# MartijnAB/guacamole

Measured on AMD Instinct MI355X. Metric: pileup loci/sec at 30x WGS; achieved HBM GB/s vs roofline, higher is better.
Workload: dtype u8; 1 GPU; germline-threshold, synthetic 30x chr20-length shard per GPU (configs[1]); genome_loci=63025519, visited_loci_per_gpu=63025483, reads_per_gpu=12612887, contigs_per_gpu=1, read_len=150, threshold=8, parallelism=loci-sharded x1

## Files before the change

guacamole_amd/csrc/gq_germline_direct.h:

```cpp
#pragma once

#include "gq_kernels.h"


#ifndef GQ_DIR_WPE
#define GQ_DIR_WPE 4
#endif
#ifndef GQ_DIR_MASKED
#define GQ_DIR_MASKED 0
#endif
#ifndef GQ_DIR_EVPF
#define GQ_DIR_EVPF 0
#endif
#ifndef GQ_DIR_U
#define GQ_DIR_U 4
#endif
struct DirCfg {
  static constexpr int kT = 512;
  static constexpr int kWaves = 4;
  static constexpr int kThreads = 64 * kWaves;
  static constexpr int kU = GQ_DIR_U;
  static constexpr int kRound = 64;
  static constexpr int kSlots = 256;
  static constexpr int64_t kMaxWin = 65535;
  static constexpr int64_t kShallow = 255;
};


template <bool DEEP>
__global__ __launch_bounds__(DirCfg::kThreads) __attribute__((amdgpu_waves_per_eu(GQ_DIR_WPE))) void germline_direct(
    const Tile *__restrict__ tiles, int64_t n_tiles, DevReads R, int threshold, int emit_ref, int emit_no_call,
    CallRec *__restrict__ recs, ComplexItem *__restrict__ cplx, OutGeom og, Counters *ctr, int32_t *__restrict__ slow,
    int32_t *__restrict__ deep, int dbg) {
  using C = DirCfg;
  constexpr int T = C::kT, U = C::kU;
  constexpr int EW = DEEP ? 2 * T : T;
  __shared__ __attribute__((aligned(16))) uint32_t evw[C::kWaves][EW];
  __shared__ __attribute__((aligned(16))) uint32_t mkw[C::kWaves][T];
  __shared__ __attribute__((aligned(16))) uint32_t dlw[C::kWaves][T];
  __shared__ __attribute__((aligned(16))) uint2 rcw[C::kWaves][C::kSlots];
  __shared__ int32_t hxw[C::kWaves][64], hnw[C::kWaves][64];
  __shared__ unsigned outn[2];
  const int lane = threadIdx.x & 63;
  const int wave = __builtin_amdgcn_readfirstlane((int)(threadIdx.x >> 6));
  uint32_t *ev = evw[wave], *mk = mkw[wave], *dl = dlw[wave];
  uint2 *rc = rcw[wave];
  int32_t *hx = hxw[wave], *hn = hnw[wave];
  auto ix = [](int32_t x) { return ((x & 7) << 6) | (x >> 3); };
  auto zero_words = [&]() {
    const uint4 z4 = make_uint4(0u, 0u, 0u, 0u);
    uint4 *e4 = reinterpret_cast<uint4 *>(ev), *m4 = reinterpret_cast<uint4 *>(mk), *d4 = reinterpret_cast<uint4 *>(dl);
#pragma unroll
    for (int q = 0; q < EW / 256; ++q) e4[64 * q + lane] = z4;
    m4[lane] = z4; m4[64 + lane] = z4; d4[lane] = z4; d4[64 + lane] = z4;
  };
  zero_words();
  if (threadIdx.x < 2) outn[threadIdx.x] = 0;
  __syncthreads();
  const int64_t per = n_tiles / gridDim.x, extra = n_tiles % gridDim.x;
  const int64_t i0 = blockIdx.x * per + min((int64_t)blockIdx.x, extra);
  const int64_t i1 = i0 + per + ((int64_t)blockIdx.x < extra ? 1 : 0);
  const int part = DEEP ? kPartsCols + (int)((blockIdx.x * C::kWaves + wave) & (kPartsWalk - 1)) : (int)blockIdx.x;
  const unsigned long long obase[2] = {og.slot(0, part, 0), og.slot(1, part, 0)};
  const unsigned long long ocap[2] = {og.cap(0, part), og.cap(1, part)};
  auto reserve = [&](int which, unsigned n) -> unsigned long long {
    return DEEP ? wave_reserve(&ctr->part[which][part], n) : (unsigned long long)wave_reserve_lds_n(outn + which, n);
  };
  unsigned visited = 0, amb = 0, ties = 0;
  uint64_t clk[8] = {0, 0, 0, 0, 0, 0, 0, 0};
  const bool multi_sample = R.n_samples > 1;
  const int64_t thr1 = (int64_t)threshold + 1;
  const uint32_t thr1u = (uint32_t)(thr1 < 0 ? 0 : thr1 > 101 ? 101 : thr1);
  const uint32_t thr1b = thr1u & 0xFFu;
  auto passes = [=](uint32_t count, uint32_t depth) { return (count & 0xFFFFu) * 100u >= thr1b * (depth & 0xFFFFu); };
  const __amdgpu_buffer_rsrc_t trs =
      __builtin_amdgcn_make_buffer_rsrc((void *)tiles, (short)0, (int)(64 * n_tiles), 0x00020000);
  const uint32_t tvo = lane < 16 ? 4u * (uint32_t)lane : 0x80000000u;
  auto fetch = [&](int64_t t) -> uint32_t { return __builtin_amdgcn_raw_buffer_load_b32(trs, (int)tvo, (int)(64 * t), 0); };
  auto f32 = [](uint32_t rec, int d) { return (uint32_t)__builtin_amdgcn_readlane((int)rec, d); };
  auto f64 = [&](uint32_t rec, int d) { return (int64_t)((uint64_t)f32(rec, d) | ((uint64_t)f32(rec, d + 1) << 32)); };
  const int32_t colr = 8 * lane;
  const int64_t n_deep = DEEP ? (int64_t)min(ctr->n_deep, (unsigned long long)n_tiles) : 0;
  const int64_t iend = DEEP ? n_deep : i1, istep = DEEP ? (int64_t)gridDim.x * C::kWaves : C::kWaves;
  int64_t i = DEEP ? (int64_t)blockIdx.x * C::kWaves + wave : i0 + wave;
  for (; i < iend; i += istep) {
    const uint64_t t_a = (dbg & 16) ? __builtin_readcyclecounter() : 0;
    const int64_t tid = DEEP ? (int64_t)__builtin_amdgcn_readfirstlane(deep[i]) : i;
    const uint32_t rec = fetch(tid);
    const int64_t ord0 = f64(rec, 0);
    const int32_t tcontig = (int32_t)f32(rec, 6);
    const int32_t L0 = (int32_t)f32(rec, 7), L1 = (int32_t)f32(rec, 8);
    const int64_t rb = f64(rec, 2), re = f64(rec, 4);
    const int32_t B0 = L0 & ~(T - 1);
    const int32_t col = B0 + colr;
    if (re <= rb) continue;
    if (re - rb > C::kMaxWin) {
      if (lane == 0) slow[atomicAdd(&ctr->n_slow, 1ull)] = (int32_t)tid;
      continue;
    }
    if (!DEEP && re - rb > C::kShallow) {
      if (lane == 0) deep[atomicAdd(&ctr->n_deep, 1ull)] = (int32_t)tid;
      continue;
    }
    uint32_t ca[2] = {0, 0}, cc[2] = {0, 0}, ct[2] = {0, 0}, cg[2] = {0, 0}, cn[2] = {0, 0};
    uint32_t wA[4] = {0, 0, 0, 0}, wC[4] = {0, 0, 0, 0}, wT[4] = {0, 0, 0, 0}, wG[4] = {0, 0, 0, 0},
             wN[4] = {0, 0, 0, 0};
    uint32_t nac[2] = {0, 0}, ntg[2] = {0, 0};
    int nn = 0, since = 0;
    auto fold = [&]() {
#pragma unroll
      for (int h = 0; h < 2; ++h) {
        ca[h] += nac[h] & 0x0F0F0F0Fu;
        cc[h] += (nac[h] >> 4) & 0x0F0F0F0Fu;
        ct[h] += ntg[h] & 0x0F0F0F0Fu;
        cg[h] += (ntg[h] >> 4) & 0x0F0F0F0Fu;
        nac[h] = ntg[h] = 0;
      }
      nn = 0;
    };
    auto widen = [&]() {
      if (!DEEP) return;
      auto w2 = [](uint32_t (&w)[4], uint32_t (&c)[2]) {
#pragma unroll
        for (int h = 0; h < 2; ++h) {
          w[2 * h] += __builtin_amdgcn_perm(0u, c[h], 0x0c010c00u);
          w[2 * h + 1] += __builtin_amdgcn_perm(0u, c[h], 0x0c030c02u);
          c[h] = 0;
        }
      };
      w2(wA, ca);
      w2(wC, cc);
      w2(wT, ct);
      w2(wG, cg);
      w2(wN, cn);
    };
    bool bad = false;
    uint32_t badb = 0;
    const uint64_t t_b = (dbg & 16) ? __builtin_readcyclecounter() : 0;
    struct Fields {
      int32_t s, e, nmd, ld;
      int64_t so, mo;
    };
    auto load_fields = [&](int64_t c0) {
      Fields f{0, 0, 0, 0, 0, 0};
      const int64_t r = c0 + lane;
      if (r < re) {
        f.s = R.start[r];
        f.e = R.end[r];
        f.so = R.seq_off[r];
        f.ld = R.lead[r];
        f.nmd = R.n_md[r];
        f.mo = R.md_off[r];
      }
      return f;
    };
    int64_t tbase = 0;
    bool defer = false;
    __amdgpu_buffer_rsrc_t srs;
    Fields nf = load_fields(rb);
    int64_t c0 = rb;
    bool first_round = true;
    uint32_t pv4[4] = {0u, 0u, 0u, 0u};
    int64_t pv_c0 = -1;
    while (c0 < re) {
      const uint64_t t_round = (dbg & 16) ? __builtin_readcyclecounter() : 0;
      hx[lane] = -1;
      hn[lane] = 0x7FFFFFFF;
      int32_t nslot = 0;
      while (c0 < re) {
        const uint64_t t_rd = (dbg & 16) ? __builtin_readcyclecounter() : 0;
        const int64_t r = c0 + lane;
        const bool valid = r < re;
        const Fields f = nf;
        const int32_t s = f.s, e = f.e, nmd = f.nmd, ld = f.ld;
        const int64_t so = f.so, mo = f.mo;
        const bool nomd = valid && nmd < 0;
        const bool gen = valid && !nomd && ld < 0;
        uint32_t nrun = valid && !nomd && !gen && e > B0 && s < B0 + T ? 1u : 0u;
        const bool evr = valid && !nomd && nmd > 0 && s < B0 + T && !(dbg & 64);
        uint32_t v4[4] = {0u, 0u, 0u, 0u};
        auto load_ev = [&](int32_t k0) {
#pragma unroll
          for (int j = 0; j < 4; ++j) v4[j] = R.md_ev[mo + (k0 + j < nmd ? k0 + j : nmd - 1)];
        };
        auto ev_add = [&](int32_t l, uint8_t base) {
          const int cat = base_cat(base);
          if (cat < 4) {
            const int32_t x = ix(l - B0);
            if (DEEP) atomicAdd(&ev[(cat >> 1) * T + x], 1u << (16 * (cat & 1)));
            else atomicAdd(&ev[x], 1u << (8 * cat));
          }
        };
        if (evr) {
          if (GQ_DIR_EVPF && pv_c0 == c0) {
#pragma unroll
            for (int j = 0; j < 4; ++j) v4[j] = pv4[j];
          } else {
            load_ev(0);
          }
        }
        if (gen && e > B0 && s < B0 + T) nrun = (uint32_t)min(-1 - ld, C::kSlots);
        const uint32_t incl = wave_incl_scan(nrun);
        const int32_t total = (int32_t)__builtin_amdgcn_readlane((int)incl, 63);
        const uint64_t t_f = (dbg & 16) ? __builtin_readcyclecounter() : 0;
        if (nslot > 0 && nslot + total > C::kSlots) break;
        if (total > C::kSlots) {
          bad = true;
          c0 = re;
          break;
        }
        if (c0 + C::kRound < re) nf = load_fields(c0 + C::kRound);
        if (first_round) {
          int64_t so_min = valid ? so : INT64_MAX;
#pragma unroll
          for (int d = 1; d < 64; d <<= 1) {
            const int64_t o = __shfl_xor(so_min, d, 64);
            so_min = o < so_min ? o : so_min;
          }
          const bool headed = R.seq_head >= 8 && so_min >= 0;
          defer = !DEEP && so_min < 8 && !headed;
          tbase = so_min >= 8 || headed ? so_min - 8 : 0;
          tbase = (int64_t)(((uint64_t)(uint32_t)__builtin_amdgcn_readfirstlane((int)(uint32_t)((uint64_t)tbase >> 32)) << 32) |
                            (uint32_t)__builtin_amdgcn_readfirstlane((int)(uint32_t)(uint64_t)tbase));
          const int64_t span = R.seq_cap - tbase;
          srs = __builtin_amdgcn_make_buffer_rsrc((void *)(R.seq + tbase), (short)0,
                                                  (int)(span < 0x7FFFFFFF ? span : 0x7FFFFFFF), 0x00020000);
          first_round = false;
        }
        bad = bad || nomd ||
              (valid && (so < tbase || so + (ld > 0 ? ld : 0) + (e > s ? e - s : 0) + 16384 + 1024 - tbase >= 0x7FFFFFF0ll));
        int32_t slot = nslot + (int32_t)(incl - nrun);
        auto put = [&](int32_t a, int32_t b, int64_t p) {
          const int32_t s16 = min(max(a - B0, -32768), 32767), e16 = min(max(b - B0, -32768), 32767);
          const int32_t K = (int32_t)(p - tbase - (int64_t)(a - B0));
          rc[slot] = make_uint2((uint32_t)(uint16_t)s16 | ((uint32_t)(uint16_t)e16 << 16), (uint32_t)K);
          atomicMax(&hx[min(max(s16, 0), T - 1) >> 3], slot);
          atomicMin(&hn[min(max(e16 - 1, 0), T - 1) >> 3], slot);
          ++slot;
// ... 323 lines not shown
```

guacamole_amd/csrc/gq_host.h:

```cpp
#pragma once
#include <hip/hip_runtime.h>

#include <algorithm>
#include <cstddef>
#include <cstring>
#include <condition_variable>
#include <mutex>
#include <thread>
#include <cstdarg>
#include <cstdio>
#include <string>
#include <utility>
#include <vector>

#include "../../include/gqpileup.h"
#include "gq_kernels.h"

namespace gq {

gq_status set_err(gq_status s, const char *fmt, ...);

#define HIP_TRY(expr)                                                                         \
  do {                                                                                        \
    hipError_t _e = (expr);                                                                   \
    if (_e != hipSuccess)                                                                     \
      return set_err(GQ_E_HIP, "%s failed: %s (%s:%d)", #expr, hipGetErrorString(_e), __FILE__, __LINE__); \
  } while (0)

constexpr int kBlock = 256;
constexpr int kGermT = 512;
constexpr int kCountT = 512;
constexpr size_t kSeqPad = 2048;

constexpr size_t kSeqHead = 16;

constexpr int kSpread = 64;
constexpr int kPartsCols = 2048;
constexpr int kPartsWalk = 1024;
constexpr int kParts = kPartsCols + kPartsWalk;

struct Counters {
  unsigned long long n_rec;
  unsigned long long n_complex;
  unsigned long long visited;
  unsigned long long ambiguous;
  unsigned long long ties;
  unsigned long long pool_used;
  int err;
  int pad;
  long long err_pos;
  unsigned long long n_slow;
  unsigned long long n_dead;
  unsigned long long part_max[2];
  unsigned long long n_amb;
  unsigned long long n_ord;
  unsigned long long n_deep;
  unsigned long long n_wide;
  unsigned long long n_gdeep[3];
  unsigned long long deep_max;
  unsigned long long deep_nt;
  unsigned long long n_out;
  unsigned long long out_pool;
  unsigned long long spread[4][64];
  unsigned long long prof[8];
  unsigned long long part[2][kParts];
  unsigned long long part_off[2][kParts + 1];
};
constexpr size_t kCountersHead = offsetof(Counters, part);

__device__ __forceinline__ unsigned long long wave_reserve(unsigned long long *ctr, unsigned n) {
  if (__ballot(n != 0) == 0) return 0;
  const int lane = threadIdx.x & 63;
  unsigned x = n;
#pragma unroll
  for (int d = 1; d < 64; d <<= 1) {
    unsigned y = __shfl_up(x, d, 64);
    if (lane >= d) x += y;
  }
  const unsigned total = __shfl(x, 63, 64);
  unsigned long long base = 0;
  if (lane == 63 && total) base = atomicAdd(ctr, (unsigned long long)total);
  base = __shfl(base, 63, 64);
  return base + (x - n);
}

struct OutGeom {
  int ncols;
  int pad_;
  unsigned long long capA[2], capB[2];
  __host__ __device__ __forceinline__ unsigned long long cap(int which, int p) const {
    return p < kPartsCols ? capA[which] : capB[which];
  }
  __host__ __device__ __forceinline__ unsigned long long slot(int which, int p, unsigned long long k) const {
    return p < kPartsCols ? (unsigned long long)p * capA[which] + k
                          : (unsigned long long)ncols * capA[which] + (unsigned long long)(p - kPartsCols) * capB[which] + k;
  }
  __host__ __device__ __forceinline__ unsigned long long total(int which) const {
    return (unsigned long long)ncols * capA[which] + (unsigned long long)(kParts - kPartsCols) * capB[which];
  }
};

__device__ __forceinline__ unsigned long long part_slot(const unsigned long long *off, unsigned long long k,
                                                        const OutGeom &g, int which) {
  int lo = 0, hi = kParts - 1;
  while (lo < hi) {
    const int m = (lo + hi + 1) >> 1;
    if (off[m] <= k) lo = m;
    else hi = m - 1;
  }
  return g.slot(which, lo, k - off[lo]);
}

template <class P>
__device__ __forceinline__ int64_t wave_first_true(int64_t lo, int64_t hi, P &&pred) {
  const int lane = threadIdx.x & 63;
  while (hi - lo > 64) {
    const int64_t step = (hi - lo + 63) / 64;
    const int64_t p = lo + (int64_t)lane * step;
    const unsigned long long b = __ballot(p >= hi || pred(p));
    if (!b) {
      lo = lo + 63 * step + 1;
      continue;
    }
    const int f = __ffsll((long long)b) - 1;
    if (f == 0) return lo;
    const int64_t nhi = lo + (int64_t)f * step;
    lo = lo + (int64_t)(f - 1) * step + 1;
    hi = nhi < hi ? nhi : hi;
  }
  const int64_t p = lo + lane;
  const unsigned long long b = __ballot(p >= hi || pred(p));
  return b ? lo + (__ffsll((long long)b) - 1) : hi;
}

template <class P1, class P2>
__device__ __forceinline__ void wave_first_true2(int64_t lo, int64_t hi, P1 &&pred1, P2 &&pred2, int64_t &out1,
                                                 int64_t &out2) {
  const int lane = threadIdx.x & 63;
  int64_t lo1 = lo, hi1 = hi, lo2 = lo, hi2 = hi;
  bool done1 = false, done2 = false;
  auto round = [&](int64_t &l, int64_t &h, bool &done, int64_t &out, bool hit) {
    if (done) return;
    if (h - l > 64) {
      const int64_t step = (h - l + 63) / 64;
      const unsigned long long b = __ballot(hit);
      if (!b) {
        l = l + 63 * step + 1;
        return;
      }
      const int f = __ffsll((long long)b) - 1;
      if (f == 0) {
        out = l;
        done = true;
        return;
      }
      const int64_t nh = l + (int64_t)f * step;
      l = l + (int64_t)(f - 1) * step + 1;
      h = nh < h ? nh : h;
    } else {
      const unsigned long long b = __ballot(hit);
      out = b ? l + (__ffsll((long long)b) - 1) : h;
      done = true;
    }
  };
  while (!(done1 && done2)) {
    const int64_t s1 = hi1 - lo1 > 64 ? (hi1 - lo1 + 63) / 64 : 1, s2 = hi2 - lo2 > 64 ? (hi2 - lo2 + 63) / 64 : 1;
    const int64_t p1 = lo1 + (int64_t)lane * s1, p2 = lo2 + (int64_t)lane * s2;
    const bool h1 = !done1 && (p1 >= hi1 || pred1(p1));
    const bool h2 = !done2 && (p2 >= hi2 || pred2(p2));
    round(lo1, hi1, done1, out1, h1);
    round(lo2, hi2, done2, out2, h2);
  }
}

__device__ __forceinline__ unsigned long long part_slot_wave(const unsigned long long *off, unsigned long long k,
                                                             const OutGeom &g, int which) {
  constexpr int kStep = (kParts + 63) / 64;
  const int lane = threadIdx.x & 63;
  const int q1 = lane * kStep;
  const bool le1 = q1 < kParts && off[q1 < kParts ? q1 : 0] <= k;
  const int base = (63 - __clzll((long long)__ballot(le1))) * kStep;
  const int q2 = base + lane;
  const bool le2 = lane < kStep && q2 < kParts && off[q2 < kParts ? q2 : 0] <= k;
  const int q = base + (63 - __clzll((long long)__ballot(le2)));
  return g.slot(which, q, k - off[q]);
}

__device__ __forceinline__ int64_t wave_id() {
  return (int64_t)blockIdx.x * (blockDim.x >> 6) + __builtin_amdgcn_readfirstlane((int)(threadIdx.x >> 6));
}

__device__ __forceinline__ uint32_t wave_incl_scan(uint32_t v) {
  v += (uint32_t)__builtin_amdgcn_update_dpp(0, (int)v, 0x111, 0xF, 0xF, true);
  v += (uint32_t)__builtin_amdgcn_update_dpp(0, (int)v, 0x112, 0xF, 0xF, true);
  v += (uint32_t)__builtin_amdgcn_update_dpp(0, (int)v, 0x114, 0xF, 0xF, true);
  v += (uint32_t)__builtin_amdgcn_update_dpp(0, (int)v, 0x118, 0xF, 0xF, true);
  v += (uint32_t)__builtin_amdgcn_update_dpp(0, (int)v, 0x142, 0xA, 0xF, false);
  v += (uint32_t)__builtin_amdgcn_update_dpp(0, (int)v, 0x143, 0xC, 0xF, false);
  return v;
}

struct SliceWin {
  int32_t c, qc0;
  int64_t ra, rz;
};
__device__ __forceinline__ SliceWin slice_window(const DevReads &R, int64_t slot) {
  int lo = 0, hi = R.n_contigs - 1;
  while (lo < hi) {
    const int m = (lo + hi + 1) >> 1;
    if (R.qoff[m] <= slot) lo = m;
    else hi = m - 1;
  }
  const int c = lo;
  const int32_t q = (int32_t)(slot - R.qoff[c]);
  const int32_t L = 128 * q;
  const int64_t cb = R.contig_read_begin[c], ce = R.contig_read_begin[c + 1];
  int64_t a0 = cb, a1 = ce;
  if (R.blk_rb) {
    const int64_t g = slot >> 2;
// ... 842 lines not shown
```

guacamole_amd/csrc/gq_pileup.hip:

```cpp
#include <hip/hip_runtime.h>
#include <hipcub/hipcub.hpp>

#include <algorithm>
#include <chrono>
#include <cstdarg>
#include <cstdlib>
#include <cstdio>
#include <cstring>
#include <string>
#include <thread>
#include <vector>

#include "../../include/gqpileup.h"
#include "gq_host.h"
#include "gq_alleles.h"

using namespace gq;

namespace {
constexpr int kScanT = 256, kScanV = 16, kScanTile = kScanT * kScanV;

__device__ __forceinline__ void scan_load16(const uint32_t *__restrict__ in, int64_t n, int64_t i0, uint32_t (&v)[kScanV]) {
  if (i0 + kScanV <= n) {
    const uint4 *p = reinterpret_cast<const uint4 *>(in + i0);
// ... 2164 lines not shown
  out->n_rows = d->n_rows;
  out->proj_reads = d->proj_reads;
  out->h2d_ms = d->h2d_ms;
  out->derive_ms = d->derive_ms;
  out->cigar_len = d->d.cigar_len;
  out->md_len = d->d.md_len;
  out->n_contigs = d->d.n_contigs;
  out->n_samples = d->d.n_samples;
  out->proj_ms = d->proj_ms;
  out->projected = d->projected ? 1 : 0;
  out->fill_ms = d->fill_ms;
  out->proj_dev_ms = d->proj_dev_ms;
  out->derive_dev_ms = d->derive_dev_ms;
  return GQ_OK;
}

void gq_reads_free(gq_dev_reads *d) {
  if (!d) return;
  if (d->ctx) (void)hipSetDevice(d->ctx->device);
  for (hipEvent_t e : d->tev)
    if (e) {
      (void)hipEventSynchronize(e);
      (void)hipEventDestroy(e);
    }
  for (void *p : d->owned) (void)hipFree(p);
  if (d->vflag) (void)hipHostFree(d->vflag);
  d->dp.free_all();
  delete d;
}

}

static int gq_dbg() {
  static const int d = getenv("GQ_DBG") ? atoi(getenv("GQ_DBG")) : 0;
  return d;
}

gq_status gq::plan(gq_ctx *c, const gq_dev_reads *rd, const gq_loci *loci, int T, Plan &pl, DevBuf &tiles_buf,
                   int stage_cap, int meta_cap, int ev_cap, bool aligned) {
  if (!loci || loci->n_ranges < 0) return set_err(GQ_E_ARG, "bad loci");
  const int64_t R = loci->n_ranges;
  pl = Plan{};
  pl.T = T;
  pl.aligned = aligned;
  std::vector<int32_t> &rc = pl.rc;
  std::vector<int64_t> &rs = pl.rs, &re = pl.re, &rt = pl.rt, ro;
  int64_t ord = 0, tiles = 0;
  for (int64_t i = 0; i < R; ++i) {
    const int32_t cc = loci->contig[i];
    const int64_t s = loci->start[i], e = loci->end[i];
    if (cc < 0 || cc >= rd->d.n_contigs) return set_err(GQ_E_ARG, "loci range %lld: contig %d out of range", (long long)i, cc);
    if (s < 0 || e < s || e > INT32_MAX) return set_err(GQ_E_ARG, "loci range %lld: bad interval", (long long)i);
    if (e == s) continue;
    const int64_t task = loci->task ? loci->task[i] : 0;
    if (pl.wins.empty() || pl.rtask.back() != task || rc.back() != cc) {
      pl.wins.push_back(Plan::Win{cc, (int64_t)rc.size(), (int64_t)rc.size()});
    } else if (s < re.back()) {
      return set_err(GQ_E_ARG, "loci range %lld: ranges of one task and contig must be sorted and disjoint",
                     (long long)i);
    }
    pl.wins.back().r1 = (int64_t)rc.size() + 1;
    pl.rwin.push_back((int32_t)(pl.wins.size() - 1));
    pl.rtask.push_back(task);
    rc.push_back(cc);
    rs.push_back(s);
    re.push_back(e);
    ro.push_back(ord);
    rt.push_back(tiles);
    ord += e - s;
    tiles += aligned ? (e - 1) / T - s / T + 1 : (e - s + T - 1) / T;
  }
  pl.n_tiles = tiles;
  pl.n_loci = ord;
  if (tiles == 0) return GQ_OK;
  const size_t nr = rc.size(), nw = pl.wins.size();
  const size_t o_rs = (nr * 4 + 15) & ~(size_t)15, o_wroff = o_rs + 4 * 8 * nr, o_rwin = o_wroff + 8 * (nw + 1),
               o_wc = o_rwin + ((4 * nr + 15) & ~(size_t)15), bytes = o_wc + 4 * nw;
  HIP_TRY(c->ranges.ensure(bytes + 64));
  char *base = (char *)c->ranges.p;
  int32_t *d_rc = (int32_t *)base;
  int64_t *d_rs = (int64_t *)(base + o_rs);
  int64_t *d_re = d_rs + nr, *d_ro = d_re + nr, *d_rt = d_ro + nr;
  {
    HIP_TRY(c->pinned(bytes));
    char *hb = (char *)c->pin;
    memcpy(hb, rc.data(), nr * 4);
    memcpy(hb + o_rs, rs.data(), nr * 8);
    memcpy(hb + o_rs + 8 * nr, re.data(), nr * 8);
    memcpy(hb + o_rs + 16 * nr, ro.data(), nr * 8);
    memcpy(hb + o_rs + 24 * nr, rt.data(), nr * 8);
    int64_t *wroff = (int64_t *)(hb + o_wroff);
    int32_t *wc = (int32_t *)(hb + o_wc);
    for (size_t w = 0; w < nw; ++w) {
      wroff[w] = pl.wins[w].r0;
      wc[w] = pl.wins[w].contig;
    }
    wroff[nw] = (int64_t)nr;
    memcpy(hb + o_rwin, pl.rwin.data(), nr * 4);
    HIP_TRY(hipMemcpyAsync(base, hb, bytes, hipMemcpyHostToDevice, c->stream));
  }
  pl.d_rs = d_rs;
  pl.d_re = d_re;
  pl.d_wroff = (const int64_t *)(base + o_wroff);
  pl.d_rwin = (const int32_t *)(base + o_rwin);
  pl.d_wcontig = (const int32_t *)(base + o_wc);
  const bool with_x = aligned && T == 512 && rd->d.srow != nullptr;
  HIP_TRY(tiles_buf.ensure((size_t)tiles * (sizeof(Tile) + (with_x ? sizeof(TileX) : 0))));
  const int nb = (int)((tiles + kBlock - 1) / kBlock);
  hipLaunchKernelGGL(plan_tiles, dim3(nb), dim3(kBlock), 0, c->stream, d_rc, d_rs, d_re, d_ro, d_rt, (int64_t)nr,
                     tiles, T, rd->d, (Tile *)tiles_buf.p, stage_cap, meta_cap, ev_cap, aligned ? 1 : 0,
                     with_x ? (TileX *)((Tile *)tiles_buf.p + tiles) : (TileX *)nullptr);
  HIP_TRY(hipGetLastError());
  return GQ_OK;
}

gq_status gq::check_device_error(gq_ctx *c, const Counters &h) {
  if (h.err == 1 && h.prof[4])
    fprintf(stderr, "gq: record slot %lld (k %llu of %llu): key %llx contig %d pos %d flags/gt %llx\n",
            (long long)h.err_pos, h.prof[3], h.prof[4], h.prof[0], (int)(h.prof[1] >> 32), (int)(uint32_t)h.prof[1],
            h.prof[2]);
  if (h.err) {
    static const char *names[] = {"ok", "assertion", "invalid cigar element", "CIGAR / MD tag mismatch",
                                  "read without MD tag", "multiple reference bases", "unsorted", "argument", "hip",
                                  "nomem", "allele table capacity"};
    const char *nm = (h.err >= 0 && h.err <= 10) ? names[h.err] : "?";
    return set_err((gq_status)h.err, "device error: %s near position %lld", nm, (long long)h.err_pos);
  }
  return GQ_OK;
}

extern "C" {

static bool germline_direct_mode(const DevReads &R) {
  static const char *m = getenv("GQ_GERM");
  static const bool proj = m && strcmp(m, "proj") == 0;
  return !proj && R.seq_cap >= 8;
}

static unsigned germline_grid(gq_ctx *c, int64_t tiles, bool direct) {
  if (c->n_cu <= 0 && hipDeviceGetAttribute(&c->n_cu, hipDeviceAttributeMultiprocessorCount, c->device) != hipSuccess)
    c->n_cu = 256;
  int &per_cu = direct ? c->dir_wg_per_cu : c->proj_wg_per_cu;
  if (per_cu <= 0) {
    int nb = 0;
    const hipError_t e = direct ? hipOccupancyMaxActiveBlocksPerMultiprocessor(&nb, germline_direct<false>, DirCfg::kThreads, 0)
                                : hipOccupancyMaxActiveBlocksPerMultiprocessor(&nb, germline_proj, ProjCfg::kThreads, 0);
    if (e != hipSuccess || nb <= 0) nb = 2;
    per_cu = nb;
  }
  const int64_t want = (tiles + ProjCfg::kWaves - 1) / ProjCfg::kWaves;
  return (unsigned)std::max<int64_t>(1, std::min<int64_t>({want, (int64_t)per_cu * c->n_cu, (int64_t)kPartsCols}));
}

static gq_status launch_germline(gq_ctx *c, int64_t tiles, const DevReads &R, const gq_germline_params *p,
                                 CallRec *recs, ComplexItem *cplx, const OutGeom &og, Counters *ctr, bool direct) {
  static const int dbg = getenv("GQ_DBG") ? atoi(getenv("GQ_DBG")) : 0;
  HIP_TRY(c->slow.ensure((size_t)tiles * sizeof(int32_t)));
  if (tiles >= (int64_t)1 << 24) return set_err(GQ_E_ARG, "%lld tiles in one call (at most 2^24)", (long long)tiles);
  if (direct) {
    HIP_TRY(c->deep_tiles.ensure((size_t)tiles * sizeof(int32_t)));
    hipLaunchKernelGGL(germline_direct<false>, dim3((unsigned)og.ncols), dim3(DirCfg::kThreads), 0, c->stream,
                       (const Tile *)c->tiles.p, tiles, R, p->threshold, p->emit_ref, p->emit_no_call, recs, cplx, og, ctr,
                       (int32_t *)c->slow.p, (int32_t *)c->deep_tiles.p, dbg);
    HIP_TRY(hipGetLastError());
    hipLaunchKernelGGL(germline_direct<true>, dim3((unsigned)std::min<int64_t>((tiles + DirCfg::kWaves - 1) / DirCfg::kWaves, 512)),
                       dim3(DirCfg::kThreads), 0, c->stream, (const Tile *)c->tiles.p, tiles, R, p->threshold,
                       p->emit_ref, p->emit_no_call, recs, cplx, og, ctr, (int32_t *)c->slow.p,
                       (int32_t *)c->deep_tiles.p, dbg);
  } else {
    hipLaunchKernelGGL(germline_proj, dim3((unsigned)og.ncols), dim3(ProjCfg::kThreads), 0, c->stream,
                       (const Tile *)c->tiles.p, (const TileX *)((const Tile *)c->tiles.p + tiles), tiles, R.proj,
                       R.pev, R.n_samples,
                       p->threshold, p->emit_ref, p->emit_no_call, recs, cplx, og, ctr, (int32_t *)c->slow.p, dbg);
  }
  HIP_TRY(hipGetLastError());
  HIP_TRY(hipEventRecord(c->ev[5], c->stream));
  const unsigned wblocks = (unsigned)std::min<int64_t>(tiles, 2048);
  hipLaunchKernelGGL((germline_walk<ProjCfg::kT>), dim3(wblocks), dim3(kBlock), 0, c->stream,
                     (const Tile *)c->tiles.p, (const int32_t *)c->slow.p, R, p->threshold, p->emit_ref,
                     p->emit_no_call, recs, cplx, og, ctr);
  HIP_TRY(hipGetLastError());
  return GQ_OK;
}

static gq_status germline_run(gq_ctx *c, const gq_dev_reads *rd, const gq_loci *loci, const gq_germline_params *p,
                              gq_calls **out, gq_calls_device *dev) {
  if (!c || !rd || !loci || !p || !out) return set_err(GQ_E_ARG, "gq_germline_threshold: null argument");
  HIP_TRY(hipSetDevice(c->device));
  const int T = c->germ_tile;
  c->timings = gq_timings{};
  const auto h0 = std::chrono::steady_clock::now();
  HIP_TRY(hipEventRecord(c->ev[0], c->stream));
  Plan pl;
  const bool direct = germline_direct_mode(rd->d);
  gq_status st = direct ? GQ_OK : ensure_projection(c, rd);
  if (st) return st;
  st = plan(c, rd, loci, T, pl, c->tiles, 0, 0, 0, true);
  if (st) return st;
  HIP_TRY(hipEventRecord(c->ev[1], c->stream));
  gq_calls *res = (gq_calls *)calloc(1, sizeof(gq_calls));
  if (!res) return set_err(GQ_E_NOMEM, "calloc");
  if (pl.n_tiles == 0) {
    st = validation_wait(rd);
    if (st) {
      free(res);
      return st;
    }
    *out = res;
    return GQ_OK;
  }
  const int ns = rd->d.n_samples;
  OutGeom og{};
  og.ncols = (int)germline_grid(c, pl.n_tiles, direct);
  const bool dense = p->emit_ref || p->emit_no_call;
  const unsigned long long wg_loci = (unsigned long long)((pl.n_tiles + og.ncols - 1) / og.ncols) * T;
  og.capA[0] = dense ? 2ull * ns * wg_loci + 64 : wg_loci / 32 + 256;
  og.capA[1] = wg_loci / 32 + 256;
  og.capB[0] = dense ? 2ull * ns * (unsigned long long)pl.n_loci / 8192 + 256 : (unsigned long long)pl.n_loci / 16384 + 256;
  og.capB[1] = (unsigned long long)pl.n_loci / 16384 + 256;
  unsigned long long pool_cap = 1 << 22, amb_cap = 4096;
  unsigned long long gdeep_cap = 1024;
  Counters hc{};
  const int bshift = dense ? 0 : 9;
  const uint64_t dead_key = ((uint64_t)pl.n_loci << 12) | 0xFFFu;
  const int64_t nbk = (pl.n_loci >> bshift) + 1;
  size_t scan_tmp = 0;
  HIP_TRY(hipcub::DeviceScan::ExclusiveSum(nullptr, scan_tmp, (const uint32_t *)nullptr, (uint32_t *)nullptr,
                                           (int)(nbk + 1), c->stream));
  const size_t fin_off = (sizeof(Counters) + 15) & ~(size_t)15;
  const size_t fin_words = 2 * (size_t)kImgBlocks + 3 * (size_t)(nbk + 1);
  auto finalize = [&](Counters *ctr, size_t cap_rec, bool cleared) -> gq_status {
    unsigned long long *bsum = (unsigned long long *)((char *)ctr + fin_off);
    uint32_t *cnt = (uint32_t *)(bsum + kImgBlocks), *off = cnt + (nbk + 1), *fill = off + (nbk + 1);
    if (!cleared)
      hipLaunchKernelGGL(zero_u32, dim3((unsigned)std::min<int64_t>(((int64_t)fin_words + kBlock - 1) / kBlock, 1024)),
                         dim3(kBlock), 0, c->stream, (uint32_t *)bsum, (int64_t)fin_words);
    const unsigned gb = (unsigned)std::max<int64_t>(1, std::min<int64_t>(((int64_t)cap_rec + kBlock - 1) / kBlock, kFinBlocks));
    hipLaunchKernelGGL(bucket_count, dim3(gb), dim3(kBlock), 0, c->stream, (const CallRec *)c->recs.p,
                       ctr, og, dead_key, bshift, nbk, (uint64_t *)c->keys.p, (int32_t *)c->idx_sorted.p,
                       (int64_t *)c->idx.p, cnt);
    HIP_TRY(hipGetLastError());
    HIP_TRY(hipcub::DeviceScan::ExclusiveSum(c->sort_tmp.p, scan_tmp, cnt, off, (int)(nbk + 1), c->stream));
    hipLaunchKernelGGL(bucket_scatter, dim3(gb), dim3(kBlock), 0, c->stream, (const Counters *)ctr,
                       (const int64_t *)c->idx.p, (const uint32_t *)off, fill, (int32_t *)c->keys_sorted.p);
    HIP_TRY(hipGetLastError());
    hipLaunchKernelGGL(bucket_rank, dim3(gb), dim3(kBlock), 0, c->stream, nbk, (const uint32_t *)off,
                       (const int32_t *)c->keys_sorted.p, (const uint64_t *)c->keys.p, (const int32_t *)c->idx_sorted.p,
                       (const int64_t *)c->idx.p, (int32_t *)c->recs_sorted.p);
    HIP_TRY(hipGetLastError());
    hipLaunchKernelGGL(img_sums, dim3(kImgBlocks), dim3(kBlock), 0, c->stream, (const CallRec *)c->recs.p,
                       (const int32_t *)c->recs_sorted.p, (const uint32_t *)off, nbk, bsum);
    hipLaunchKernelGGL(calls_image, dim3(kImgBlocks), dim3(kBlock), 0, c->stream, (const CallRec *)c->recs.p,
                       (const int32_t *)c->recs_sorted.p, (const uint32_t *)off, nbk, (const unsigned long long *)bsum,
                       (const uint8_t *)c->pool.p, ctr, (uint8_t *)c->image.p);
    HIP_TRY(hipGetLastError());
    return GQ_OK;
  };
  auto read_counters = [&](Counters *ctr) -> gq_status {
    HIP_TRY(c->pinned(kCountersHead));
    HIP_TRY(hipMemcpyAsync(c->pin, ctr, kCountersHead, hipMemcpyDeviceToHost, c->stream));
    HIP_TRY(hipStreamSynchronize(c->stream));
    memcpy(&hc, c->pin, kCountersHead);
    return GQ_OK;
  };
  for (int attempt = 0; attempt < 3; ++attempt) {
    HIP_TRY(c->amb.ensure(2 * amb_cap * sizeof(AmbItem)));
    const size_t cap_rec = (size_t)og.total(0);
    HIP_TRY(c->recs.ensure(cap_rec * sizeof(CallRec)));
    HIP_TRY(c->cplx.ensure(og.total(1) * sizeof(ComplexItem)));
    HIP_TRY(c->pool.ensure(pool_cap));
    HIP_TRY(c->counters.ensure(fin_off + 4 * fin_words));
    HIP_TRY(c->keys.ensure((cap_rec + 1) * 8));
    HIP_TRY(c->keys_sorted.ensure((cap_rec + 1) * 4));
    HIP_TRY(c->idx.ensure((cap_rec + 1) * 8));
    HIP_TRY(c->idx_sorted.ensure((cap_rec + 1) * 4));
    HIP_TRY(c->recs_sorted.ensure((cap_rec + 1) * 4));
    HIP_TRY(c->sort_tmp.ensure(std::max<size_t>(scan_tmp, 16)));
    HIP_TRY(c->image.ensure(calls_layout((int64_t)cap_rec, (int64_t)pool_cap).bytes));
    Counters *ctr = (Counters *)c->counters.p;
    HIP_TRY(hipMemsetAsync(ctr, 0, fin_off + 4 * fin_words, c->stream));
    if (attempt == 0) HIP_TRY(hipEventRecord(c->ev[1], c->stream));
    st = launch_germline(c, pl.n_tiles, rd->d, p, (CallRec *)c->recs.p, (ComplexItem *)c->cplx.p, og, ctr, direct);
    if (st) {
      free(res);
      return st;
    }
    HIP_TRY(hipEventRecord(c->ev[2], c->stream));
#ifndef GQ_CPLX_BLOCKS
#define GQ_CPLX_BLOCKS 4096
#endif
    const int cblocks = (int)std::min<int64_t>(std::max<int64_t>(pl.n_tiles, 1), GQ_CPLX_BLOCKS);
    SomWin wb{};
    st = window_bounds(c, pl, rd, wb);
    if (st) {
      free(res);
      return st;
    }
    hipLaunchKernelGGL(part_scan, dim3(1), dim3(1024), 0, c->stream, ctr, 1, og);
    HIP_TRY(c->deep_list.ensure(3 * sizeof(int64_t) * (size_t)gdeep_cap));
    auto complex_pair = [&](int blocks, int which, AmbItem *amb_out, unsigned long long acap, const AmbItem *amb_in,
                            const uint8_t *amb_ref, int64_t n_amb_in, const SomWin &sw_) -> gq_status {
      int64_t *region = (int64_t *)c->deep_list.p + (size_t)which * gdeep_cap;
      const DeepList fast{region, &ctr->n_gdeep[which], nullptr, nullptr, gdeep_cap};
      const DeepList wide{nullptr, nullptr, region, &ctr->n_gdeep[which], gdeep_cap};
      hipLaunchKernelGGL(germline_complex<2>, dim3(blocks), dim3(kBlock), 0, c->stream, (const Tile *)c->tiles.p,
                         (const ComplexItem *)c->cplx.p, rd->d, p->threshold, p->emit_ref, p->emit_no_call,
                         (CallRec *)c->recs.p, og, (uint8_t *)c->pool.p, pool_cap, ctr, amb_out, acap, amb_in, amb_ref,
                         n_amb_in, gq_dbg(), sw_, fast);
      HIP_TRY(hipGetLastError());
      hipLaunchKernelGGL(germline_complex<16>, dim3(64), dim3(kBlock), 0, c->stream, (const Tile *)c->tiles.p,
                         (const ComplexItem *)c->cplx.p, rd->d, p->threshold, p->emit_ref, p->emit_no_call,
                         (CallRec *)c->recs.p, og, (uint8_t *)c->pool.p, pool_cap, ctr, amb_out, acap, amb_in, amb_ref,
                         n_amb_in, gq_dbg(), sw_, wide);
      HIP_TRY(hipGetLastError());
      return GQ_OK;
    };
    st = complex_pair(cblocks, 0, (AmbItem *)c->amb.p, amb_cap, (const AmbItem *)nullptr, (const uint8_t *)nullptr,
                      (int64_t)0, wb);
    if (st) {
      free(res);
      return st;
    }
    {
#ifndef GQ_EXPAND_BLOCKS
#define GQ_EXPAND_BLOCKS 1024
#endif
      hipLaunchKernelGGL(germline_expand, dim3(GQ_EXPAND_BLOCKS), dim3(kBlock), 0, c->stream, (CallRec *)c->recs.p, ctr, og,
                         p->threshold, p->emit_ref, p->emit_no_call, dead_key);
      HIP_TRY(hipGetLastError());
    }
    HIP_TRY(hipEventRecord(c->ev[3], c->stream));
    st = finalize(ctr, cap_rec, true);
    if (st) {
      free(res);
      return st;
    }
    HIP_TRY(hipEventRecord(c->ev[4], c->stream));
    st = read_counters(ctr);
    if (!st) st = validation_settled(rd);
    if (st) {
      free(res);
      return st;
    }
    bool retry = false;
    for (int w = 0; w < 2; ++w)
      if (hc.part_max[w]) {
        og.capA[w] += hc.part_max[w] + 64;
        og.capB[w] += hc.part_max[w] + 64;
        retry = true;
      }
    if (hc.pool_used > pool_cap) {
      pool_cap = hc.pool_used + 4096;
      retry = true;
    }
    if (hc.n_amb > amb_cap || hc.n_ord > amb_cap) {
      amb_cap = std::max(hc.n_amb, hc.n_ord) + 1024;
      retry = true;
    }
    if (hc.n_gdeep[0] > gdeep_cap) {
      gdeep_cap = hc.n_gdeep[0] + 1024;
      retry = true;
    }
    SomWin sw{};
    const bool rerun = !retry && (hc.n_amb > 0 || hc.n_ord > 0) && !hc.err;
    if (rerun) {
      st = build_somwin(c, pl, rd, rd, sw);
      if (st) {
        free(res);
        return st;
      }
    }
    if (rerun && hc.n_ord > 0) {
      const int oblocks = (int)std::min<int64_t>(((int64_t)hc.n_ord + 3) / 4, 4096);
      st = complex_pair(oblocks, 1, (AmbItem *)nullptr, (unsigned long long)0, (const AmbItem *)c->amb.p + amb_cap,
                        (const uint8_t *)nullptr, (int64_t)hc.n_ord, sw);
      if (st) {
        free(res);
        return st;
      }
      hipLaunchKernelGGL(part_scan, dim3(1), dim3(1024), 0, c->stream, ctr, 0, og);
    }
    if (rerun && hc.n_amb > 0) {
      std::vector<AmbItem> amb((size_t)hc.n_amb);
      HIP_TRY(hipMemcpyAsync(amb.data(), c->amb.p, amb.size() * sizeof(AmbItem), hipMemcpyDeviceToHost, c->stream));
      HIP_TRY(hipStreamSynchronize(c->stream));
      HIP_TRY(c->amb_ref.ensure(amb.size()));
      st = heap_ref_bases(c, pl, c->tiles, {rd}, amb, (uint8_t *)c->amb_ref.p);
      if (st) {
        free(res);
        return st;
      }
      const int ablocks = (int)std::min<int64_t>(((int64_t)amb.size() + 3) / 4, 4096);
      st = complex_pair(ablocks, 2, (AmbItem *)nullptr, (unsigned long long)0, (const AmbItem *)c->amb.p,
                        (const uint8_t *)c->amb_ref.p, (int64_t)amb.size(), sw);
      if (st) {
        free(res);
        return st;
      }
      hipLaunchKernelGGL(part_scan, dim3(1), dim3(1024), 0, c->stream, ctr, 0, og);
    }
    if (rerun) {
      HIP_TRY(hipEventRecord(c->ev[3], c->stream));
      st = read_counters(ctr);
      if (st) {
        free(res);
        return st;
      }
      if (hc.part_max[0]) {
        og.capA[0] += hc.part_max[0] + 64;
        og.capB[0] += hc.part_max[0] + 64;
        retry = true;
      }
      if (hc.pool_used > pool_cap) {
        pool_cap = hc.pool_used + 4096;
        retry = true;
      }
      if (std::max(hc.n_gdeep[1], hc.n_gdeep[2]) > gdeep_cap) {
        gdeep_cap = std::max(hc.n_gdeep[1], hc.n_gdeep[2]) + 1024;
        retry = true;
      }
      if (!retry) {
        st = finalize(ctr, cap_rec, false);
        if (!st) {
          HIP_TRY(hipEventRecord(c->ev[4], c->stream));
          st = read_counters(ctr);
        }
        if (st) {
          free(res);
          return st;
        }
      }
    }
    if (!retry) break;
    if (attempt == 2) {
      free(res);
      return set_err(GQ_E_CAPACITY, "output capacity retries exhausted");
    }
  }
  if ((gq_dbg() & 32) && hc.prof[4])
    fprintf(stderr, "gq germline_complex prof (cycles/item/wave): cover %.0f reference-base %.0f elements %.0f "
            "map-order %.0f decision %.0f (%llu items)\n", (double)hc.prof[0] / hc.prof[4],
            (double)hc.prof[1] / hc.prof[4], (double)hc.prof[2] / hc.prof[4], (double)hc.prof[5] / hc.prof[4],
            (double)hc.prof[3] / hc.prof[4], hc.prof[4]);
  if ((gq_dbg() & 16) && hc.prof[5])
    fprintf(stderr,
            "gq prof (cycles/tile/wave): setup %.0f chunks %.0f (runs %.0f [fields %.0f slots %.0f] counting %.0f) "
            "decision %.0f (%llu)\n",
            (double)hc.prof[0] / hc.prof[5], (double)hc.prof[1] / hc.prof[5], (double)hc.prof[2] / hc.prof[5],
            (double)hc.prof[6] / hc.prof[5], (double)hc.prof[7] / hc.prof[5], (double)hc.prof[3] / hc.prof[5],
            (double)hc.prof[4] / hc.prof[5], hc.prof[5]);
  for (int k = 0; k < kSpread; ++k) {
    hc.visited += hc.spread[0][k];
    hc.ambiguous += hc.spread[1][k];
    hc.ties += hc.spread[2][k];
    hc.n_dead += hc.spread[3][k];
  }
  st = check_device_error(c, hc);
  if (st) {
    free(res);
    return st;
  }
  const int64_t n = (int64_t)hc.n_out;
  const CallsLayout lay = calls_layout(n, (int64_t)hc.out_pool);
  const int64_t pool_len = (int64_t)hc.out_pool;
  uint8_t *blk = nullptr;
  if (dev) {
    blk = (uint8_t *)c->image.p;
    dev->image = c->image.p;
    dev->image_bytes = (int64_t)lay.pool + pool_len;
  } else {
    const size_t nbytes = (size_t)lay.pool + (size_t)pool_len;
    blk = (uint8_t *)malloc(std::max<size_t>(nbytes, 64));
    if (!blk) {
      free(res);
      return set_err(GQ_E_NOMEM, "result block of %zu bytes", nbytes);
    }
    HIP_TRY(hipMemcpyAsync(blk, c->image.p, nbytes, hipMemcpyDeviceToHost, c->stream));
    HIP_TRY(hipStreamSynchronize(c->stream));
  }
  const auto h1 = std::chrono::steady_clock::now();
  res->n = n;
  res->block_ = dev ? nullptr : blk;
  res->contig = (int32_t *)(blk + lay.contig);
  res->pos = (int64_t *)(blk + lay.pos);
  res->ref_off = (int64_t *)(blk + lay.ref_off);
  res->alt_off = (int64_t *)(blk + lay.alt_off);
  res->ref_len = (int32_t *)(blk + lay.ref_len);
  res->alt_len = (int32_t *)(blk + lay.alt_len);
  res->sample = blk + lay.sample;
  res->gt0 = blk + lay.gt0;
  res->gt1 = blk + lay.gt1;
  res->flags = blk + lay.flags;
  res->allele_pool = blk + lay.pool;
  res->pool_len = pool_len;
  res->visited_loci = (int64_t)hc.visited;
  res->complex_loci = (int64_t)hc.n_complex;
  res->ambiguous_loci = (int64_t)hc.ambiguous;
  res->tie_loci = (int64_t)hc.ties;
  float ms = 0;
  (void)hipEventElapsedTime(&ms, c->ev[0], c->ev[1]);
  c->timings.plan_ms = ms;
  (void)hipEventElapsedTime(&ms, c->ev[1], c->ev[5]);
  c->timings.pileup_ms = ms;
  (void)hipEventElapsedTime(&ms, c->ev[5], c->ev[2]);
  c->timings.walk_ms = ms;
  c->timings.walk_tiles = (int64_t)hc.n_slow;
  c->timings.order_loci = (int64_t)hc.n_ord;
  (void)hipEventElapsedTime(&ms, c->ev[2], c->ev[3]);
  c->timings.complex_ms = ms;
  (void)hipEventElapsedTime(&ms, c->ev[3], c->ev[4]);
  c->timings.finalize_ms = ms;
  (void)hipEventElapsedTime(&ms, c->ev[0], c->ev[4]);
  c->timings.total_ms = ms;
  c->timings.pileup_launches = 1;
  c->timings.tiles = pl.n_tiles;
  const auto h2 = std::chrono::steady_clock::now();
  c->timings.host_ms = std::chrono::duration<float, std::milli>(h2 - h0).count();
  c->timings.marshal_ms = std::chrono::duration<float, std::milli>(h2 - h1).count();
  *out = res;
  return GQ_OK;
}

gq_status gq_germline_threshold(gq_ctx *c, const gq_dev_reads *rd, const gq_loci *loci,
                                const gq_germline_params *p, gq_calls **out) {
  return germline_run(c, rd, loci, p, out, nullptr);
}

gq_status gq_germline_threshold_device(gq_ctx *c, const gq_dev_reads *rd, const gq_loci *loci,
                                       const gq_germline_params *p, gq_calls_device *out) {
  if (!out) return set_err(GQ_E_ARG, "gq_germline_threshold_device: null argument");
  memset(out, 0, sizeof(*out));
  gq_calls *r = nullptr;
  const gq_status st = germline_run(c, rd, loci, p, &r, out);
  if (st) return st;
  out->calls = *r;
  out->calls.block_ = nullptr;
  free(r);
  return GQ_OK;
}

gq_status gq_write_vcf_germline(const char *path, const char *header, int64_t n, const int32_t *contig,
                                const int64_t *pos, const uint8_t *gt0, const uint8_t *gt1, const int64_t *ref_off,
                                const int32_t *ref_len, const int64_t *alt_off, const int32_t *alt_len,
                                const uint8_t *pool, int32_t n_contigs, const char *const *contig_names) {
  if (!path || !header || (n > 0 && (!contig || !pos || !gt0 || !gt1 || !ref_off || !ref_len || !alt_off || !alt_len ||
                                      !contig_names)))
    return set_err(GQ_E_ARG, "gq_write_vcf_germline: null argument");
  FILE *f = fopen(path, "wb");
  if (!f) return set_err(GQ_E_ARG, "cannot write %s", path);
  std::string buf(header);
  buf.reserve((size_t)n * 48 + buf.size() + 64);
  static const char kGt[4] = {'0', '1', '.', '.'};
  std::vector<size_t> clen((size_t)std::max(n_contigs, 0));
  for (int32_t k = 0; k < n_contigs; ++k) clen[(size_t)k] = contig_names[k] ? strlen(contig_names[k]) : 0;
  char num[24];
  bool ok = true;
  for (int64_t i = 0; i < n && ok; ++i) {
    const int32_t c = contig[i];
    if (c < 0 || c >= n_contigs || !contig_names[c]) {
      fclose(f);
      return set_err(GQ_E_ARG, "gq_write_vcf_germline: record %lld has contig %d", (long long)i, c);
    }
    buf.append(contig_names[c], clen[(size_t)c]);
    buf += '\t';
    const int k = snprintf(num, sizeof num, "%lld", (long long)(pos[i] + 1));
    buf.append(num, (size_t)k);
    buf.append("\t.\t", 3);
    buf.append((const char *)pool + ref_off[i], (size_t)ref_len[i]);
    buf += '\t';
    buf.append((const char *)pool + alt_off[i], (size_t)alt_len[i]);
    buf.append("\t.\t.\t.\tGT\t", 10);
    buf += kGt[gt0[i] & 3];
    buf += '/';
    buf += kGt[gt1[i] & 3];
    buf += '\n';
    if (buf.size() > (size_t)(64 << 20)) {
      ok = fwrite(buf.data(), 1, buf.size(), f) == buf.size();
      buf.clear();
    }
  }
  if (ok && !buf.empty()) ok = fwrite(buf.data(), 1, buf.size(), f) == buf.size();
  if (fclose(f) != 0) ok = false;
  return ok ? GQ_OK : set_err(GQ_E_ARG, "write to %s failed", path);
}

void gq_free_calls(gq_calls *r) {
  if (!r) return;
// ... 384 lines not shown
```

Measured before the change: 38.38 billion loci/s.

## Schedule shallow germline tiles dynamically via sharded atomic work heads

Replaces the static per-block tile range in the shallow germline_direct kernel with dynamic work claiming from eight atomic tile heads. Each wave prefetches its next claim one tile ahead, and once its own head is exhausted it steals from the other heads. This targets load imbalance across waves and blocks, at the cost of extra atomics. Because output partitions were sized for a static assignment, the change also adds a retry attempt that falls back to static scheduling when partition capacity overflows.

```diff
diff --git a/guacamole_amd/csrc/gq_germline_direct.h b/guacamole_amd/csrc/gq_germline_direct.h
--- a/guacamole_amd/csrc/gq_germline_direct.h
+++ b/guacamole_amd/csrc/gq_germline_direct.h
@@ -15,6 +15,9 @@
 #ifndef GQ_DIR_U
 #define GQ_DIR_U 4
 #endif
+#ifndef GQ_DIR_G
+#define GQ_DIR_G 1
+#endif
 struct DirCfg {
   static constexpr int kT = 512;
   static constexpr int kWaves = 4;
@@ -27,7 +30,7 @@
 };
 
 
-template <bool DEEP>
+template <bool DEEP, bool HAND = false>
 __global__ __launch_bounds__(DirCfg::kThreads) __attribute__((amdgpu_waves_per_eu(GQ_DIR_WPE))) void germline_direct(
     const Tile *__restrict__ tiles, int64_t n_tiles, DevReads R, int threshold, int emit_ref, int emit_no_call,
     CallRec *__restrict__ recs, ComplexItem *__restrict__ cplx, OutGeom og, Counters *ctr, int32_t *__restrict__ slow,
@@ -81,9 +84,51 @@
   auto f64 = [&](uint32_t rec, int d) { return (int64_t)((uint64_t)f32(rec, d) | ((uint64_t)f32(rec, d + 1) << 32)); };
   const int32_t colr = 8 * lane;
   const int64_t n_deep = DEEP ? (int64_t)min(ctr->n_deep, (unsigned long long)n_tiles) : 0;
-  const int64_t iend = DEEP ? n_deep : i1, istep = DEEP ? (int64_t)gridDim.x * C::kWaves : C::kWaves;
+  int64_t iend = DEEP ? n_deep : i1, istep = DEEP ? (int64_t)gridDim.x * C::kWaves : C::kWaves;
   int64_t i = DEEP ? (int64_t)blockIdx.x * C::kWaves + wave : i0 + wave;
-  for (; i < iend; i += istep) {
+  static_assert(!(DEEP && HAND), "the deep instantiation walks its list");
+  constexpr bool hand = HAND;
+  int hd = (int)(blockIdx.x & (kTileHeads - 1)), heads_left = kTileHeads;
+  uint32_t ahead = 0;
+  bool claimed = false;
+  auto claim = [&]() {
+    uint32_t k = 0;
+    if (lane == 0)
+      k = __hip_atomic_fetch_add(&ctr->tile_head[hd][0], (unsigned)GQ_DIR_G, __ATOMIC_RELAXED, __HIP_MEMORY_SCOPE_AGENT);
+    return k;
+  };
+  auto next_group = [&]() -> bool {
+    while (heads_left > 0) {
+      const int64_t lo = (n_tiles * hd) / kTileHeads, n = (n_tiles * (hd + 1)) / kTileHeads - lo;
+      uint32_t k;
+      if (claimed) {
+        k = (uint32_t)__builtin_amdgcn_readfirstlane((int)ahead);
+        claimed = false;
+      } else {
+        k = (uint32_t)__builtin_amdgcn_readfirstlane(
+            (int)__hip_atomic_load(&ctr->tile_head[hd][0], __ATOMIC_RELAXED, __HIP_MEMORY_SCOPE_AGENT));
+        if ((int64_t)k < n) k = (uint32_t)__builtin_amdgcn_readfirstlane((int)claim());
+      }
+      if ((int64_t)k < n) {
+        i = lo + k;
+        iend = min(i + GQ_DIR_G, lo + n);
+        return true;
+      }
+      hd = (hd + 1) & (kTileHeads - 1);
+      --heads_left;
+    }
+    return false;
+  };
+  if (hand) {
+    i = iend = 0;
+    istep = 1;
+  }
+  for (;; i += istep) {
+    if (i >= iend && !(hand && next_group())) break;
+    if (hand && i + 1 >= iend) {
+      ahead = claim();
+      claimed = true;
+    }
     const uint64_t t_a = (dbg & 16) ? __builtin_readcyclecounter() : 0;
     const int64_t tid = DEEP ? (int64_t)__builtin_amdgcn_readfirstlane(deep[i]) : i;
     const uint32_t rec = fetch(tid);
diff --git a/guacamole_amd/csrc/gq_host.h b/guacamole_amd/csrc/gq_host.h
--- a/guacamole_amd/csrc/gq_host.h
+++ b/guacamole_amd/csrc/gq_host.h
@@ -38,6 +38,7 @@
 constexpr int kPartsCols = 2048;
 constexpr int kPartsWalk = 1024;
 constexpr int kParts = kPartsCols + kPartsWalk;
+constexpr int kTileHeads = 8;
 
 struct Counters {
   unsigned long long n_rec;
@@ -65,6 +66,7 @@
   unsigned long long prof[8];
   unsigned long long part[2][kParts];
   unsigned long long part_off[2][kParts + 1];
+  alignas(128) unsigned tile_head[kTileHeads][32];
 };
 constexpr size_t kCountersHead = offsetof(Counters, part);
 
diff --git a/guacamole_amd/csrc/gq_pileup.hip b/guacamole_amd/csrc/gq_pileup.hip
--- a/guacamole_amd/csrc/gq_pileup.hip
+++ b/guacamole_amd/csrc/gq_pileup.hip
@@ -2340,16 +2340,23 @@
   return (unsigned)std::max<int64_t>(1, std::min<int64_t>({want, (int64_t)per_cu * c->n_cu, (int64_t)kPartsCols}));
 }
 
+static int germline_tile_sched() {
+  const char *m = getenv("GQ_TILES");
+  return m && strcmp(m, "static") == 0 ? 0 : 1;
+}
+
 static gq_status launch_germline(gq_ctx *c, int64_t tiles, const DevReads &R, const gq_germline_params *p,
-                                 CallRec *recs, ComplexItem *cplx, const OutGeom &og, Counters *ctr, bool direct) {
+                                 CallRec *recs, ComplexItem *cplx, const OutGeom &og, Counters *ctr, bool direct,
+                                 int sched) {
   static const int dbg = getenv("GQ_DBG") ? atoi(getenv("GQ_DBG")) : 0;
   HIP_TRY(c->slow.ensure((size_t)tiles * sizeof(int32_t)));
   if (tiles >= (int64_t)1 << 24) return set_err(GQ_E_ARG, "%lld tiles in one call (at most 2^24)", (long long)tiles);
   if (direct) {
     HIP_TRY(c->deep_tiles.ensure((size_t)tiles * sizeof(int32_t)));
-    hipLaunchKernelGGL(germline_direct<false>, dim3((unsigned)og.ncols), dim3(DirCfg::kThreads), 0, c->stream,
-                       (const Tile *)c->tiles.p, tiles, R, p->threshold, p->emit_ref, p->emit_no_call, recs, cplx, og, ctr,
-                       (int32_t *)c->slow.p, (int32_t *)c->deep_tiles.p, dbg);
+    const auto shallow = sched ? germline_direct<false, true> : germline_direct<false, false>;
+    hipLaunchKernelGGL(shallow, dim3((unsigned)og.ncols),
+                       dim3(DirCfg::kThreads), 0, c->stream, (const Tile *)c->tiles.p, tiles, R, p->threshold, p->emit_ref,
+                       p->emit_no_call, recs, cplx, og, ctr, (int32_t *)c->slow.p, (int32_t *)c->deep_tiles.p, dbg);
     HIP_TRY(hipGetLastError());
     hipLaunchKernelGGL(germline_direct<true>, dim3((unsigned)std::min<int64_t>((tiles + DirCfg::kWaves - 1) / DirCfg::kWaves, 512)),
                        dim3(DirCfg::kThreads), 0, c->stream, (const Tile *)c->tiles.p, tiles, R, p->threshold,
@@ -2451,7 +2458,9 @@
     memcpy(&hc, c->pin, kCountersHead);
     return GQ_OK;
   };
-  for (int attempt = 0; attempt < 3; ++attempt) {
+  int max_attempts = 3;
+  for (int attempt = 0; attempt < max_attempts; ++attempt) {
+    const int sched = direct && !dense && attempt == 0 ? germline_tile_sched() : 0;
     HIP_TRY(c->amb.ensure(2 * amb_cap * sizeof(AmbItem)));
     const size_t cap_rec = (size_t)og.total(0);
     HIP_TRY(c->recs.ensure(cap_rec * sizeof(CallRec)));
@@ -2468,7 +2477,7 @@
     Counters *ctr = (Counters *)c->counters.p;
     HIP_TRY(hipMemsetAsync(ctr, 0, fin_off + 4 * fin_words, c->stream));
     if (attempt == 0) HIP_TRY(hipEventRecord(c->ev[1], c->stream));
-    st = launch_germline(c, pl.n_tiles, rd->d, p, (CallRec *)c->recs.p, (ComplexItem *)c->cplx.p, og, ctr, direct);
+    st = launch_germline(c, pl.n_tiles, rd->d, p, (CallRec *)c->recs.p, (ComplexItem *)c->cplx.p, og, ctr, direct, sched);
     if (st) {
       free(res);
       return st;
@@ -2536,6 +2545,7 @@
         og.capA[w] += hc.part_max[w] + 64;
         og.capB[w] += hc.part_max[w] + 64;
         retry = true;
+        if (sched != 0) max_attempts = 4;
       }
     if (hc.pool_used > pool_cap) {
       pool_cap = hc.pool_used + 4096;
@@ -2598,6 +2608,7 @@
         og.capA[0] += hc.part_max[0] + 64;
         og.capB[0] += hc.part_max[0] + 64;
         retry = true;
+        if (sched != 0) max_attempts = 4;
       }
       if (hc.pool_used > pool_cap) {
         pool_cap = hc.pool_used + 4096;
@@ -2620,7 +2631,7 @@
       }
     }
     if (!retry) break;
-    if (attempt == 2) {
+    if (attempt + 1 == max_attempts) {
       free(res);
       return set_err(GQ_E_CAPACITY, "output capacity retries exhausted");
     }
```

New measurement: 41.30 billion loci/s, median of 6. +7.6%, better.
